# UMich-CURLY/SE3ET

Measured on AMD Instinct MI355X. Metric: point-cloud pairs/sec (fwd), SE3ET-E 5k-pt pairs, higher is better.
Workload: dtype f32

## Files before the change

include/se3et_hip.h:

```cpp
#ifndef SE3ET_HIP_H_
#define SE3ET_HIP_H_

#include <stddef.h>
#include <stdint.h>

#ifdef __cplusplus
extern "C" {
#endif

#define SE3_OK 0
#define SE3_ERR_INVALID_ARG 1
#define SE3_ERR_UNSUPPORTED 2
#define SE3_ERR_LAUNCH 3
#define SE3_ERR_WORKSPACE 4

#define SE3_MAX_BATCH 32
#define SE3_MAX_NEIGHBOR_LIMIT 64

const char* se3_version(void);
const char* se3_last_error(void);
void se3_debug_set_sinkhorn_variant(int variant);
unsigned long long se3_debug_dense_saturated_rows(int reset);
unsigned long long se3_debug_attention_saturated(int reset);
void se3_debug_kernel_timing(int enable);
int se3_debug_kernel_timing_collect_ex(float* microseconds, int* tags, double* aux, int capacity);

int se3_radius_neighbors(const float* q_points, int64_t nq, const float* s_points, int64_t ns,
                         const int64_t* q_lengths_host, const int64_t* s_lengths_host, int batch, float radius,
                         int limit, int64_t* neighbors, int32_t* max_count, void* stream);

int se3_neighbor_table_trim(const int64_t* full, int64_t rows, int full_width, int width, const int64_t* pair_row_ends_host,
                            const int* pair_widths_host, int num_pairs, int64_t* out, void* stream);
size_t se3_radius_grid_workspace_bytes(int64_t ns, int batch);
int se3_radius_grid_build(const float* s_points, int64_t ns, const int64_t* s_lengths_host, int batch, float radius,
                          void* workspace, size_t workspace_bytes, void* stream);
int se3_radius_neighbors_grid(const float* q_points, int64_t nq, const int64_t* q_lengths_host, const int64_t* s_lengths_host,
                              int64_t ns, int batch, const void* grid_workspace, float radius, int limit, int64_t* neighbors,
                              int32_t* max_count, int max_count_is_zero, void* stream);

int se3_radius_count_hist(const float* q_points, int64_t nq, const float* s_points, int64_t ns, const int64_t* q_lengths_host,
                          const int64_t* s_lengths_host, int batch, float radius, const void* grid_workspace, int hist_n,
                          const int* slot_of_cloud_host, int num_slots, int32_t* hist, int32_t* dropped, int32_t* max_count, void* stream);

int se3_radius_neighbors_ties(const float* q_points, int64_t nq, const float* s_points, int64_t ns, const int64_t* q_lengths_host,
                              const int64_t* s_lengths_host, int batch, float radius, int limit, int64_t* neighbors, int32_t* max_count,
                              int32_t* tie_rows, int32_t* tie_count, void* stream);
int se3_radius_neighbors_grid_ties(const float* q_points, int64_t nq, const int64_t* q_lengths_host, const int64_t* s_lengths_host,
                                   int64_t ns, int batch, const void* grid_workspace, float radius, int limit, int64_t* neighbors,
                                   int32_t* max_count, int max_count_is_zero, int32_t* tie_rows, int32_t* tie_count, void* stream);
size_t se3_kdtree_max_bytes(int64_t ns, int batch);
int se3_kdtree_build_host(const float* s_points_host, int64_t ns, const int64_t* s_lengths_host, int batch, void* tree_host, size_t capacity,
                          size_t* used_bytes);
size_t se3_radius_tie_scratch_bytes(int64_t num_tie_rows, int max_hits);
int se3_radius_neighbors_tie_order(const float* q_points, int64_t nq, const float* s_points, int64_t ns, const int64_t* q_lengths_host,
                                   const int64_t* s_lengths_host, int batch, const void* tree_dev, float radius, int limit,
                                   const int32_t* tie_rows, int64_t num_tie_rows, int max_hits, void* scratch, size_t scratch_bytes,
                                   int64_t* neighbors, void* stream);
int se3_debug_radius_tie_order_host(const float* q_points, int64_t nq, const float* s_points, int64_t ns, const int64_t* q_lengths,
                                    const int64_t* s_lengths, int batch, const void* tree_host, float radius, int limit,
                                    const int32_t* tie_rows, int64_t num_tie_rows, int max_hits, int64_t* neighbors, int* overflowed);
int64_t se3_debug_std_sort_host(const unsigned long long* keys, int64_t n, int mode);

size_t se3_grid_subsample_workspace_bytes(int64_t n, int batch);
int se3_grid_subsample(const float* points, const float* normals, int64_t n, const int64_t* lengths_host, int batch,
                       float voxel_size, float* s_points, float* s_normals, int64_t* s_lengths, void* workspace,
                       size_t workspace_bytes, void* stream);
int se3_grid_subsample_dev(const float* points, const float* normals, int64_t n_rows, const int64_t* lengths_dev, int batch,
                           float voxel_size, float* s_points, float* s_normals, int64_t* s_lengths, void* workspace,
                           size_t workspace_bytes, void* stream);

int se3_log_sinkhorn_fwd(const float* scores, const uint8_t* row_masks, const uint8_t* col_masks, const float* alpha,
                         int batch, int rows, int cols, int iterations, float inf, float* out, void* stream);
int se3_log_sinkhorn_bwd(const float* scores, const uint8_t* row_masks, const uint8_t* col_masks, const float* alpha,
                         const float* grad_out, int batch, int rows, int cols, int iterations, float inf, float* grad_scores,
                         float* grad_alpha_partial, void* stream);

size_t se3_group_norm_workspace_bytes(int64_t rows, int channels, int groups);
int se3_group_norm_fwd(const float* x, const float* x_bias, const float* residual, const float* weight, const float* bias,
                       int64_t rows, int channels, int groups, float eps, int apply_leaky_relu, float slope, float* out,
                       void* workspace, size_t workspace_bytes, void* stream);

int se3_group_norm_segments_fwd(const float* x, const float* x_bias, const float* residual, const float* weight,
                                const float* bias, int64_t rows, int channels, int groups,
                                const int64_t* segment_row_offsets_host, int num_segments, float eps, int apply_leaky_relu,
                                float slope, float* out, void* workspace, size_t workspace_bytes, void* stream);
size_t se3_group_norm_bwd_workspace_bytes(int channels);
int se3_group_norm_segments_bwd(const float* x, const float* x_bias, const float* residual, const float* weight, const float* bias,
                                const float* grad_out, int64_t rows, int channels, int groups, const int64_t* segment_row_offsets_host,
                                int num_segments, float eps, int apply_leaky_relu, float slope, float* grad_x, float* grad_residual,
                                float* grad_params, void* workspace, size_t workspace_bytes, void* stream);

size_t se3_group_norm_stats_workspace_bytes(int channels);
int se3_group_norm_stats(const float* x, const float* in_affine, float in_slope, const float* x_bias, const float* weight, const float* bias,
                         int64_t rows, int channels, int groups, const int64_t* segment_row_offsets_host, int num_segments, float eps,
                         float* affine_out, void* workspace, size_t workspace_bytes, void* stream);
int se3_group_norm_apply(const float* x, const float* affine_a, float slope_a, const float* affine_b, float slope_b, const float* residual,
                         const float* residual_affine, float final_slope, int64_t rows, int channels,
                         const int64_t* segment_row_offsets_host, int num_segments, int blocked_layout, float* out, void* stream);
int se3_group_norm_apply_amax(const float* x, const float* affine_a, float slope_a, const float* affine_b, float slope_b, const float* residual,
                              const float* residual_affine, float final_slope, int64_t rows, int channels,
                              const int64_t* segment_row_offsets_host, int num_segments, int blocked_layout, float* out, float* amax_out,
                              void* stream);
size_t se3_dense_norm_workspace_bytes(int groups);
int se3_dense_norm_fwd(const float* x, int64_t rows, int in_features, const float* in_affine_a, float in_slope_a, const float* in_affine_b,
                       float in_slope_b, const void* weight_pieces, int out_features, const float* linear_bias, const float* norm_weight,
// ... 556 lines not shown
```

se3et_amd/csrc/dense_norm.hip:

```cpp
#include "common.h"
#include "group_norm.h"

namespace {

using f16x8 = __attribute__((ext_vector_type(8))) _Float16;
using f16x4 = __attribute__((ext_vector_type(4))) _Float16;
using f32x16 = __attribute__((ext_vector_type(16))) float;
using f32x4 = __attribute__((ext_vector_type(4))) float;
using u32x4 = __attribute__((ext_vector_type(4))) unsigned;
using i32x4 = __attribute__((ext_vector_type(4))) int;

__device__ unsigned long long g_dense_saturated_rows = 0;

template <int CTRL>
__device__ __forceinline__ float dpp_f32(float v) {
  return __builtin_bit_cast(float, __builtin_amdgcn_update_dpp(0, __builtin_bit_cast(int, v), CTRL, 0xf, 0xf, true));
}

constexpr int kHeaderB = 256;
constexpr int kRowB = 80;

struct DenseArgs {
  const float* x;
  const float* in_affine[2];
  float in_slope[2];
  int K, N, NCT;
  const u32x4* Wf;
  const float* hdr;
  float* out;
  float* part;
  int* counters;
  const float* xb;
  const float* gw;
  const float* gb;
  float* affine;
  int groups;
  float eps;
  SegTable T;
  const float* affine1;
  const float* residual;
  const float* x2;
  int K2;
  const u32x4* Wf2;
  const float* hdr2;
  const float* affine2;
  float final_slope;
  int x_rs, out_rs;
  int t_rows;
  int t_ld;
  int seg_steps;
  long long seg_stride;
};


struct StepPos {
  int tile, kk;
};
template <int WM, int WN, int RT, int CT, int MODE>
__global__ __launch_bounds__(256, MODE == 3 ? 2 : 3) void dense_norm_kernel(const DenseArgs a) {
  static_assert(WM * WN == 4, "4 waves");
  constexpr int TR = 32 * RT * WM, BN = 32 * CT * WN, U = TR / 32;
  constexpr int kPieceB = TR * kRowB, kBufB = 2 * kPieceB;
  constexpr bool kStats = MODE <= 1, kDual = MODE == 3, kPlain = MODE >= 4;
  __shared__ __align__(16) unsigned char lds[2 * kBufB];
  __shared__ __align__(16) int row_exp[2][TR];
  __shared__ __align__(16) int row_exp_step[2][TR];
  __shared__ int row_run[TR];
  __shared__ int row_scl[2];
  extern __shared__ __align__(16) float aff[];
  const int tid = threadIdx.x, lane = tid & 63, wave = __builtin_amdgcn_readfirstlane(tid >> 6);
  const int wm = wave / WN, wn = wave % WN;
  const int i32 = lane & 31, h = lane >> 5;
  const int K = a.K, N = a.N;
  const int K2 = kDual ? a.K2 : 32;
  const int XS = kPlain ? a.x_rs : K, OS = kPlain ? a.out_rs : N;
  long long r0, r1;
  chunk_rows(a.T, blockIdx.x, r0, r1);
  if (r1 < r0) r1 = r0;
  const int seg = seg_of_chunk(a.T, blockIdx.x);
  int cb0 = a.T.chunk_begin[0], cb1 = a.T.chunk_begin[1];
#pragma unroll
  for (int i = 1; i < kGNMaxSegments; i++)
    if (seg == i) {
// ... 396 lines not shown
  StepPos pr{0, 0}, ps{0, 0}, pm{0, 0};
  request(pr, ra);
  advance(pr);
  request(pr, rb);
  advance(pr);
  __syncthreads();
  stage(0, ps, ra);
  advance(ps);
#pragma unroll
  for (int j = 0; j < U; j++) ra[j] = rb[j];
  request(pr, rb);
  advance(pr);
  __syncthreads();
  if constexpr (WD == 1) {
#pragma unroll 1
    for (int s = 0; s < total; s++) {
      multiply(s & 1, pm, bq[0]);
      advance(pm);
      stage((s + 1) & 1, ps, ra);
      advance(ps);
#pragma unroll
      for (int j = 0; j < U; j++) ra[j] = rb[j];
      request(pr, rb);
      advance(pr);
      __syncthreads();
    }
  } else {
#pragma unroll 1
    for (int s = 0; s < total; s += WD) {
#pragma unroll
      for (int j = 0; j < WD; j++) {
        if (s + j >= total) break;
        multiply(j & 1, pm, bq[j]);
        advance(pm);
        stage((j + 1) & 1, ps, ra);
        advance(ps);
#pragma unroll
        for (int u = 0; u < U; u++) ra[u] = rb[u];
        request(pr, rb);
        advance(pr);
        __syncthreads();
      }
    }
  }
  if constexpr (!kStats) return;
  __syncthreads();
  const int cpg = N / a.groups;
  WF* sh = reinterpret_cast<WF*>(lds);
  if (a.xb)
#pragma unroll
    for (int c = 0; c < CT; c++) run[c].mean += a.xb[(ct0 + c) * 32 + i32];
  if (h == 0)
#pragma unroll
    for (int c = 0; c < CT; c++) sh[(wave * CT + c) * 32 + i32] = run[c];
  __syncthreads();
  if (wm == 0)
#pragma unroll
    for (int c = 0; c < CT; c++) {
      WF w = run[c];
      for (int m = 1; m < WM; m++) w = wf_merge(w, sh[((m * WN + wn) * CT + c) * 32 + i32]);
      for (int d = 1; d < cpg; d <<= 1) {
        const WF o = {__shfl_xor(w.n, d), __shfl_xor(w.mean, d), __shfl_xor(w.m2, d)};
        w = wf_merge(w, o);
      }
      const int col = (ct0 + c) * 32 + i32;
      if (h == 0 && (col & (cpg - 1)) == 0) gn_store_partial(a.part + ((int64_t)blockIdx.x * a.groups + col / cpg) * 3, w);
    }
  if (!gn_last_arrival(a.counters + seg * kGNMaxColumnBlocks + blockIdx.y, cb1 - cb0)) return;
  const int gpb = BN / cpg;
  gn_finalize_groups(a.part, a.groups, cb0, cb1, blockIdx.y * gpb, gpb, cpg, a.xb, a.gw, a.gb, a.eps, a.affine + (size_t)seg * 2 * N, N);
}

constexpr int kTargetChunks = 768;

}

extern "C" unsigned long long se3_debug_dense_saturated_rows(int reset) {
  unsigned long long n = 0;
  if (hipMemcpyFromSymbol(&n, HIP_SYMBOL(g_dense_saturated_rows), sizeof(n)) != hipSuccess) return ~0ull;
  if (reset) {
    const unsigned long long zero = 0;
    (void)hipMemcpyToSymbol(HIP_SYMBOL(g_dense_saturated_rows), &zero, sizeof(zero));
  }
  return n;
}

constexpr size_t kCounterB = kGNCounterB;

extern "C" size_t se3_dense_norm_workspace_bytes(int groups) {
  return kCounterB + (size_t)(kGNMaxChunks + kGNMaxSegments) * (groups > 0 ? groups : 1) * 3 * sizeof(float);
}

namespace {
int dense_chunks(int64_t rows, int N, const int64_t* segment_row_offsets_host, int num_segments, SegTable& T, int& TR, int& BN, int& ncb,
                 bool given = false) {
  if (!given) {
    TR = N >= 256 ? 64 : 128;
    BN = N >= 256 ? 256 : N;
  }
  ncb = (N + BN - 1) / BN;
  T = SegTable{};
  T.n = num_segments;
  T.quantum = TR;
  int64_t tiles = 0;
  for (int s = 0; s < num_segments; s++) {
    const int64_t b0 = num_segments == 1 ? 0 : segment_row_offsets_host[s], b1 = num_segments == 1 ? rows : segment_row_offsets_host[s + 1];
    if (!(b1 > b0 && b0 >= 0 && b1 <= rows)) return -1;
    tiles += se3_cdiv(b1 - b0, TR);
  }
  int64_t want = kTargetChunks / ncb;
  if (want > kGNMaxChunks - num_segments) want = kGNMaxChunks - num_segments;
  if (want < 1) want = 1;
  int64_t tiles_per_chunk = se3_cdiv(tiles, want);
  for (int s = 0; s < num_segments; s++) {
    const int64_t b0 = num_segments == 1 ? 0 : segment_row_offsets_host[s], b1 = num_segments == 1 ? rows : segment_row_offsets_host[s + 1];
    const int64_t need = se3_cdiv(se3_cdiv(b1 - b0, TR), 256);
    if (need > tiles_per_chunk) tiles_per_chunk = need;
  }
  int chunks = 0;
  for (int s = 0; s < num_segments; s++) {
    const int64_t b0 = num_segments == 1 ? 0 : segment_row_offsets_host[s], b1 = num_segments == 1 ? rows : segment_row_offsets_host[s + 1];
    T.row_begin[s] = b0;
    T.row_begin[s + 1] = b1;
    T.chunk_begin[s] = chunks;
    chunks += (int)se3_cdiv(se3_cdiv(b1 - b0, TR), tiles_per_chunk);
    T.chunk_begin[s + 1] = chunks;
  }
  if (!(T.row_begin[0] == 0 && T.row_begin[num_segments] == rows && chunks <= kGNMaxChunks + kGNMaxSegments)) return -1;
  return chunks;
}

template <int MODE>
void dense_launch(const DenseArgs& a, int N, dim3 grid, size_t dyn, hipStream_t st) {
  if (N >= 256) dense_norm_kernel<1, 4, 2, 2, MODE><<<grid, 256, dyn, st>>>(a);
  else if (N == 128) dense_norm_kernel<2, 2, 2, 2, MODE><<<grid, 256, dyn, st>>>(a);
  else if (N == 64) dense_norm_kernel<4, 1, 1, 2, MODE><<<grid, 256, dyn, st>>>(a);
  else dense_norm_kernel<4, 1, 1, 1, MODE><<<grid, 256, dyn, st>>>(a);
}
}

extern "C" int se3_dense_norm_fwd(const float* x, int64_t rows, int in_features, const float* in_affine_a, float in_slope_a,
                                  const float* in_affine_b, float in_slope_b, const void* weight_pieces, int out_features,
                                  const float* linear_bias, const float* norm_weight, const float* norm_bias, int groups, float eps,
                                  const int64_t* segment_row_offsets_host, int num_segments, float* out, float* affine_out, void* workspace,
                                  size_t workspace_bytes, void* stream) {
  SE3_REQUIRE(x && weight_pieces && norm_weight && norm_bias && affine_out && workspace, SE3_ERR_INVALID_ARG, "dense_norm: null pointer");
  const int K = in_features, N = out_features;
  SE3_REQUIRE(K >= 32 && K <= 1024 && (K & (K - 1)) == 0 && N >= 32 && N % 32 == 0 && (N < 256 ? (N & (N - 1)) == 0 : N % 256 == 0),
              SE3_ERR_UNSUPPORTED, "dense_norm: %d -> %d features (in: a power of two 32..1024; out: 32, 64, 128 or a multiple of 256)", K, N);
  SE3_REQUIRE(rows >= 1 && groups >= 1 && N % groups == 0, SE3_ERR_INVALID_ARG, "dense_norm: rows %lld groups %d", (long long)rows, groups);
  {
    const int cpg = N / groups;
    SE3_REQUIRE(cpg <= 32 && (cpg & (cpg - 1)) == 0 && N / (N >= 256 ? 256 : N) <= kGNMaxColumnBlocks, SE3_ERR_UNSUPPORTED,
                "dense_norm: %d channels per group (a power of two <= 32), %d output features (<= %d)", cpg, N, 256 * kGNMaxColumnBlocks);
  }
  SE3_REQUIRE(num_segments >= 1 && num_segments <= kGNMaxSegments && (num_segments == 1 || segment_row_offsets_host), SE3_ERR_UNSUPPORTED,
              "dense_norm: %d segments (1..%d)", num_segments, kGNMaxSegments);
  SE3_REQUIRE(((uintptr_t)x & 15) == 0 && (in_affine_a || !in_affine_b), SE3_ERR_INVALID_ARG, "dense_norm: x must be 16-byte aligned; stage b needs stage a");
  SE3_REQUIRE(in_slope_a >= 0.f && in_slope_a <= 1.f && in_slope_b >= 0.f && in_slope_b <= 1.f, SE3_ERR_INVALID_ARG, "dense_norm: LeakyReLU slopes must lie in [0, 1]");
  SE3_REQUIRE(workspace_bytes >= se3_dense_norm_workspace_bytes(groups), SE3_ERR_WORKSPACE, "dense_norm: workspace too small");
  SegTable T;
  int TR, BN, ncb;
  const int chunks = dense_chunks(rows, N, segment_row_offsets_host, num_segments, T, TR, BN, ncb);
  SE3_REQUIRE(chunks > 0, SE3_ERR_INVALID_ARG, "dense_norm: the segments must be non-empty, ascending and cover all %lld rows", (long long)rows);
  DenseArgs a{};
  a.x = x;
  a.in_affine[0] = in_affine_a;
  a.in_affine[1] = in_affine_b;
  a.in_slope[0] = in_slope_a;
  a.in_slope[1] = in_slope_b;
  a.K = K;
  a.N = N;
  a.NCT = (N + 63) / 64 * 2;
  a.hdr = static_cast<const float*>(weight_pieces);
  a.Wf = reinterpret_cast<const u32x4*>(static_cast<const unsigned char*>(weight_pieces) + kHeaderB);
  a.out = out;
  a.counters = static_cast<int*>(workspace);
  a.part = reinterpret_cast<float*>(static_cast<unsigned char*>(workspace) + kCounterB);
  a.xb = linear_bias;
  a.gw = norm_weight;
  a.gb = norm_bias;
  a.affine = affine_out;
  a.groups = groups;
  a.eps = eps;
  a.T = T;
  const size_t dyn = (size_t)((in_affine_a != nullptr) + (in_affine_b != nullptr)) * 2 * K * sizeof(float);
  hipStream_t st = (hipStream_t)stream;
  const dim3 grid((unsigned)chunks, (unsigned)ncb);
  if (out != nullptr) dense_launch<0>(a, N, grid, dyn, st);
  else dense_launch<1>(a, N, grid, dyn, st);
  SE3_CHECK_LAUNCH("dense_norm");
  return SE3_OK;
}

extern "C" int se3_dense_residual_fwd(const float* x, int64_t rows, int in_features, const float* in_affine_a, float in_slope_a,
                                      const float* in_affine_b, float in_slope_b, const void* weight_pieces, const float* affine,
                                      const float* x2, int in_features2, const void* weight_pieces2, const float* affine2,
                                      const float* residual, int out_features, float final_slope, const int64_t* segment_row_offsets_host,
                                      int num_segments, float* out, void* stream) {
  SE3_REQUIRE(x && weight_pieces && affine && out, SE3_ERR_INVALID_ARG, "dense_residual: null pointer");
  const int K = in_features, N = out_features, K2 = in_features2;
  SE3_REQUIRE(K >= 32 && K <= 1024 && (K & (K - 1)) == 0 && N >= 32 && N % 32 == 0 && (N < 256 ? (N & (N - 1)) == 0 : N % 256 == 0),
              SE3_ERR_UNSUPPORTED, "dense_residual: %d -> %d features (in: a power of two 32..1024; out: 32, 64, 128 or a multiple of 256)", K, N);
  SE3_REQUIRE(!(x2 && residual), SE3_ERR_INVALID_ARG, "dense_residual: a residual tensor OR a shortcut layer");
  SE3_REQUIRE(!x2 || (weight_pieces2 && affine2 && K2 >= 32 && K2 <= 1024 && (K2 & (K2 - 1)) == 0 && ((uintptr_t)x2 & 15) == 0), SE3_ERR_UNSUPPORTED,
              "dense_residual: shortcut layer with %d input features (a power of two 32..1024, 16-byte aligned rows)", K2);
  SE3_REQUIRE(rows >= 1 && num_segments >= 1 && num_segments <= kGNMaxSegments && (num_segments == 1 || segment_row_offsets_host), SE3_ERR_UNSUPPORTED,
              "dense_residual: rows %lld, %d segments (1..%d)", (long long)rows, num_segments, kGNMaxSegments);
  SE3_REQUIRE(((uintptr_t)x & 15) == 0 && (in_affine_a || !in_affine_b), SE3_ERR_INVALID_ARG, "dense_residual: x must be 16-byte aligned; stage b needs stage a");
  SE3_REQUIRE(in_slope_a >= 0.f && in_slope_a <= 1.f && in_slope_b >= 0.f && in_slope_b <= 1.f && final_slope >= 0.f && final_slope <= 1.f, SE3_ERR_INVALID_ARG,
              "dense_residual: LeakyReLU slopes must lie in [0, 1]");
  SegTable T;
  int TR, BN, ncb;
  const int chunks = dense_chunks(rows, N, segment_row_offsets_host, num_segments, T, TR, BN, ncb);
  SE3_REQUIRE(chunks > 0, SE3_ERR_INVALID_ARG, "dense_residual: the segments must be non-empty, ascending and cover all %lld rows", (long long)rows);
  DenseArgs a{};
  a.x = x;
  a.in_affine[0] = in_affine_a;
  a.in_affine[1] = in_affine_b;
  a.in_slope[0] = in_slope_a;
  a.in_slope[1] = in_slope_b;
  a.K = K;
  a.N = N;
  a.NCT = (N + 63) / 64 * 2;
  a.hdr = static_cast<const float*>(weight_pieces);
  a.Wf = reinterpret_cast<const u32x4*>(static_cast<const unsigned char*>(weight_pieces) + kHeaderB);
  a.out = out;
  a.T = T;
  a.affine1 = affine;
  a.residual = residual;
  a.final_slope = final_slope;
  const size_t dyn = (size_t)((in_affine_a != nullptr) + (in_affine_b != nullptr)) * 2 * K * sizeof(float);
  hipStream_t st = (hipStream_t)stream;
  const dim3 grid((unsigned)chunks, (unsigned)ncb);
  if (x2 != nullptr) {
    a.x2 = x2;
    a.K2 = K2;
    a.hdr2 = static_cast<const float*>(weight_pieces2);
    a.Wf2 = reinterpret_cast<const u32x4*>(static_cast<const unsigned char*>(weight_pieces2) + kHeaderB);
    a.affine2 = affine2;
    dense_launch<3>(a, N, grid, dyn, st);
  } else {
    dense_launch<2>(a, N, grid, dyn, st);
  }
  SE3_CHECK_LAUNCH("dense_residual");
  return SE3_OK;
}


namespace {
template <int WM, int WN, int RT, int CT>
void plain_launch(const DenseArgs& a, bool transposed, dim3 grid, hipStream_t st) {
  if (transposed) dense_norm_kernel<WM, WN, RT, CT, 5><<<grid, 256, 0, st>>>(a);
  else dense_norm_kernel<WM, WN, RT, CT, 4><<<grid, 256, 0, st>>>(a);
}
int linear_stream_one(const float* x, int64_t rows, int K, int64_t x_rs, const void* weight_pieces, const float* bias, int N, int relu, float* out,
                      int64_t out_rs, int t_rows, int64_t t_ld, void* stream, int seg_channels = 0, int64_t seg_stride = 0) {
  SE3_REQUIRE(x && weight_pieces && out, SE3_ERR_INVALID_ARG, "linear_stream: null pointer");
  SE3_REQUIRE(K > 0 && K % 32 == 0 && N > 0, SE3_ERR_UNSUPPORTED, "linear_stream: in_features %d must be a multiple of 32", K);
  SE3_REQUIRE(x_rs >= 4 && x_rs % 4 == 0 && ((uintptr_t)x & 15) == 0 && rows * x_rs < (1ll << 29), SE3_ERR_INVALID_ARG,
              "linear_stream: x rows must be 16-byte aligned, row stride %lld, below 2 GB", (long long)x_rs);
  const bool transposed = t_rows > 0;
  if (transposed)
    SE3_REQUIRE(t_rows % 4 == 0 && rows % t_rows == 0 && t_ld >= t_rows && t_ld % 4 == 0 && ((uintptr_t)out & 15) == 0 &&
                    (rows / t_rows) * N * t_ld < (1ll << 29),
                SE3_ERR_INVALID_ARG, "linear_stream: transposed output blocks of %d rows (a multiple of 4 dividing %lld), leading dimension %lld",
                t_rows, (long long)rows, (long long)t_ld);
  else
    SE3_REQUIRE(out_rs >= N && rows * out_rs < (1ll << 29), SE3_ERR_INVALID_ARG, "linear_stream: out row stride %lld", (long long)out_rs);
  if (rows == 0) return SE3_OK;
  int TR, BN, cfg;
  const int64_t rt64 = se3_cdiv(rows, 64);
  if (N > 128) {
    if (rt64 * se3_cdiv(N, 256) >= 512) { TR = 64; BN = 256; cfg = 0; }
    else if (rt64 * se3_cdiv(N, 128) >= 320 || N % 128 > 64) { TR = 64; BN = 128; cfg = 1; }
    else { TR = 64; BN = 64; cfg = 2; }
  } else if (N > 64) { TR = rt64 >= 512 ? 128 : 64; BN = 128; cfg = rt64 >= 512 ? 3 : 1; }
  else if (N > 32) { TR = rt64 >= 512 ? 128 : 64; BN = 64; cfg = rt64 >= 512 ? 4 : 2; }
  else { TR = 128; BN = 32; cfg = 5; }
  if (transposed && cfg == 3) { TR = 64; cfg = 1; }
  SegTable T;
  int ncb;
  const int chunks = dense_chunks(rows, N, nullptr, 1, T, TR, BN, ncb, true);
  SE3_REQUIRE(chunks > 0, SE3_ERR_INVALID_ARG, "linear_stream: %lld rows", (long long)rows);
  DenseArgs a{};
  a.x = x;
  a.K = K;
  a.N = N;
  a.NCT = (N + 63) / 64 * 2;
  a.hdr = static_cast<const float*>(weight_pieces);
  a.Wf = reinterpret_cast<const u32x4*>(static_cast<const unsigned char*>(weight_pieces) + kHeaderB);
  a.out = out;
  a.xb = bias;
  a.T = T;
  a.final_slope = relu ? 0.f : 1.f;
  a.x_rs = (int)x_rs;
  a.out_rs = (int)out_rs;
  a.t_rows = t_rows;
  a.t_ld = (int)t_ld;
  if (seg_channels > 0) {
    SE3_REQUIRE(seg_channels % 32 == 0 && K % seg_channels == 0 && seg_stride >= rows * x_rs && (K / seg_channels) * seg_stride < (1ll << 29),
                SE3_ERR_INVALID_ARG, "linear_stream: %d input channels in segments of %d", K, seg_channels);
    a.seg_steps = seg_channels / 32;
    a.seg_stride = seg_stride;
  }
  hipStream_t st = (hipStream_t)stream;
  const dim3 grid((unsigned)chunks, (unsigned)ncb);
  switch (cfg) {
    case 0: plain_launch<1, 4, 2, 2>(a, transposed, grid, st); break;
    case 1: plain_launch<2, 2, 1, 2>(a, transposed, grid, st); break;
    case 2: plain_launch<2, 2, 1, 1>(a, transposed, grid, st); break;
    case 3: plain_launch<2, 2, 2, 2>(a, transposed, grid, st); break;
    case 4: plain_launch<4, 1, 1, 2>(a, transposed, grid, st); break;
    default: plain_launch<4, 1, 1, 1>(a, transposed, grid, st); break;
  }
  SE3_CHECK_LAUNCH("linear_stream");
  return SE3_OK;
}

int linear_stream(const float* x, int64_t rows, int K, int64_t x_rs, const void* weight_pieces, const float* bias, int N, int relu, float* out,
                  int64_t out_rs, int t_rows, int64_t t_ld, void* stream, int seg_channels = 0, int64_t seg_stride = 0) {
  const int64_t lim = (1ll << 29) - 1;
  const bool transposed = t_rows > 0;
  const bool fits = rows >= 0 && x_rs > 0 && rows * x_rs <= lim &&
                    (transposed ? (rows / t_rows) * (int64_t)N * t_ld <= lim : rows * (out_rs > N ? out_rs : (int64_t)N) <= lim);
  if (fits || seg_channels > 0 || !x || !out || N <= 0) return linear_stream_one(x, rows, K, x_rs, weight_pieces, bias, N, relu, out, out_rs, t_rows, t_ld, stream, seg_channels, seg_stride);
  int64_t step;
  if (transposed) {
    SE3_REQUIRE(rows % t_rows == 0 && t_ld >= t_rows, SE3_ERR_INVALID_ARG, "linear_stream: transposed output blocks of %d rows", t_rows);
    const int64_t per_block = std::max((int64_t)t_rows * x_rs, (int64_t)N * t_ld);
    SE3_REQUIRE(per_block <= lim, SE3_ERR_UNSUPPORTED, "linear_stream: one transposed block of %d rows exceeds 2 GB", t_rows);
    step = lim / per_block * t_rows;
  } else {
    SE3_REQUIRE(out_rs >= N, SE3_ERR_INVALID_ARG, "linear_stream: out row stride %lld", (long long)out_rs);
    step = lim / std::max(x_rs, out_rs) / 256 * 256;
    SE3_REQUIRE(step > 0, SE3_ERR_UNSUPPORTED, "linear_stream: row strides %lld / %lld too large", (long long)x_rs, (long long)out_rs);
  }
  for (int64_t r0 = 0; r0 < rows; r0 += step) {
    const int64_t n = std::min(step, rows - r0);
    float* o = transposed ? out + (r0 / t_rows) * (int64_t)N * t_ld : out + r0 * out_rs;
    const int rc = linear_stream_one(x + r0 * x_rs, n, K, x_rs, weight_pieces, bias, N, relu, o, out_rs, t_rows, t_ld, stream);
    if (rc != SE3_OK) return rc;
  }
  return SE3_OK;
}
}

extern "C" int se3_linear_stream(const float* x, int64_t rows, int in_features, int64_t x_row_stride, const void* weight_pieces, const float* bias,
                                 int out_features, int apply_relu, float* out, int64_t out_row_stride, void* stream) {
  return linear_stream(x, rows, in_features, x_row_stride, weight_pieces, bias, out_features, apply_relu, out, out_row_stride, 0, 0, stream);
}

extern "C" int se3_linear_stream_transposed(const float* x, int64_t rows, int in_features, int64_t x_row_stride, const void* weight_pieces,
                                            const float* bias, int out_features, int block_rows, float* out_t, int64_t ld, void* stream) {
  SE3_REQUIRE(block_rows > 0, SE3_ERR_INVALID_ARG, "linear_stream_transposed: block_rows %d", block_rows);
  return linear_stream(x, rows, in_features, x_row_stride, weight_pieces, bias, out_features, 0, out_t, 0, block_rows, ld, stream);
}


extern "C" int se3_linear_stream_segments(const float* x, int64_t rows, int in_features, int seg_channels, int64_t seg_stride,
                                          const void* weight_pieces, const float* bias, int out_features, int apply_relu, float* out,
                                          int64_t out_row_stride, void* stream) {
  SE3_REQUIRE(seg_channels > 0, SE3_ERR_INVALID_ARG, "linear_stream_segments: seg_channels %d", seg_channels);
  return linear_stream(x, rows, in_features, seg_channels, weight_pieces, bias, out_features, apply_relu, out, out_row_stride, 0, 0, stream,
                       seg_channels, seg_stride);
}
```

se3et_amd/ops.py:

```python
import ctypes
import os
import threading

import torch

from .caches import CACHE_EPOCH, Derived, Workspace, _Shared, also_clear, clear_caches, clear_weight_caches, validate_weight_caches
from ._lib import CONSTANTS, ENUMS, check, lib
from .stacking import PAIR_MAX_PAIRS, device_offsets, exclusive_offsets, to_device


_HAS_BLAS_SWITCH = hasattr(torch.backends.cuda, 'preferred_blas_library')
if _HAS_BLAS_SWITCH:
    torch.backends.cuda.preferred_blas_library('cublas')
_BLAS_SWITCH_LOCK = threading.Lock()
_BIG_GEMM_FLOP = 2.0e9


def mm(a, b):
    big = 2.0 * a.shape[0] * a.shape[1] * b.shape[1] > _BIG_GEMM_FLOP
    if _HAS_BLAS_SWITCH and big and (b.stride(-1) == 1 or a.shape[1] <= 32):
        with _BLAS_SWITCH_LOCK:
            torch.backends.cuda.preferred_blas_library('cublaslt')
            try:
                return torch.mm(a, b)
            finally:
                torch.backends.cuda.preferred_blas_library('cublas')
    if _HAS_BLAS_SWITCH and threading.active_count() > 1:
        with _BLAS_SWITCH_LOCK:
            return torch.mm(a, b)
    return torch.mm(a, b)


LINEAR_F16_MIN_ROWS, LINEAR_F16_MIN_K = 20000, 256
_linear_pieces = Derived(512, weights=True)


def _linear_weight_pieces(weight, stream):
    N, K = weight.shape
    owner = weight._base if weight._base is not None else weight
    key = (weight.data_ptr(), N, K, weight.stride(0), weight.device.index)
    Wp = _linear_pieces.lookup(owner, key)
    if Wp is not None:
        return Wp
    Wp = torch.empty((lib().se3_linear_weight_pieces_bytes(N, K),), dtype=torch.uint8, device=weight.device)
    w = weight.detach()
    w = w if w.is_contiguous() else w.contiguous()
    check(lib().se3_linear_split_weights_f16(w.data_ptr(), N, K, Wp.data_ptr(), stream), 'se3_linear_split_weights_f16')
    return _linear_pieces.store(owner, key, Wp, fingerprint_of=(weight,))


_stacked_weights = Derived(128, weights=True)


def stacked_weight(weight, groups):
    key = (weight.data_ptr(), tuple(weight.shape), int(groups), weight.device.index)
    W = _stacked_weights.lookup(weight, key)
    if W is not None:
        return W
    with torch.no_grad():
        W = torch.cat([weight.detach()] * int(groups), 1).contiguous()
    return _stacked_weights.store(weight, key, W, fingerprint_of=(weight,))


def linear_f16_ok(x, weight):
    if torch.is_grad_enabled() and (x.requires_grad or weight.requires_grad):
        return False
    if not (x.is_cuda and x.dtype == torch.float32 and weight.dtype == torch.float32 and weight.dim() == 2 and weight.is_contiguous()):
        return False
    K = weight.shape[1]
    rows = x.numel() // max(x.shape[-1], 1)
    return (x.shape[-1] == K and K % 32 == 0 and K >= LINEAR_F16_MIN_K and rows >= LINEAR_F16_MIN_ROWS and x.is_contiguous()
            and x.data_ptr() % 16 == 0)


def linear_f16(x, weight, bias=None, relu=False):
    stream = _stream()
    N, K = weight.shape
    rows = x.numel() // K
    Wp = _linear_weight_pieces(weight, stream)
    out = torch.empty(x.shape[:-1] + (N,), dtype=torch.float32, device=x.device)
    b = None if bias is None else _req(bias.detach().contiguous(), torch.float32, 'bias', 1)
    check(lib().se3_linear_f16(x.data_ptr(), rows, K, K, Wp.data_ptr(), None if b is None else b.data_ptr(), N, 1 if relu else 0,
                               out.data_ptr(), N, stream), 'se3_linear_f16')
    return out


def dense_saturated_rows(reset=True):
    return int(lib().se3_debug_dense_saturated_rows(1 if reset else 0))


def attention_saturated(reset=True):
    return int(lib().se3_debug_attention_saturated(1 if reset else 0))


def linear_stream_ok(x, weight):
    if torch.is_grad_enabled() and (x.requires_grad or weight.requires_grad):
        return False
    if not (x.is_cuda and x.dtype == torch.float32 and weight.dtype == torch.float32 and weight.dim() == 2 and weight.stride(1) == 1):
        return False
    K = weight.shape[1]
    return x.shape[-1] == K and K % 32 == 0 and x.stride(-1) == 1 and x.data_ptr() % 16 == 0 and (x.is_contiguous() or (x.dim() == 2 and x.stride(0) % 4 == 0))


def linear_stream(x, weight, bias=None, relu=False, out=None):
    stream = _stream()
    N, K = weight.shape
    rows = x.numel() // K
    x_rs = x.stride(0) if (x.dim() == 2 and not x.is_contiguous()) else K
    Wp = _linear_weight_pieces(weight, stream)
    if out is None:
        out = torch.empty(x.shape[:-1] + (N,), dtype=torch.float32, device=x.device)
        out_rs = N
    else:
        if out.dim() != 2 or out.shape[0] != rows or out.shape[1] != N or out.stride(1) != 1 or out.dtype != torch.float32:
            raise RuntimeError('linear_stream: out must be a (rows, N) float32 view with unit column stride')
        out_rs = out.stride(0)
    b = None if bias is None else _req(bias.detach().contiguous(), torch.float32, 'bias', 1)
    check(lib().se3_linear_stream(x.data_ptr(), rows, K, x_rs, Wp.data_ptr(), None if b is None else b.data_ptr(), N, 1 if relu else 0,
                                  out.data_ptr(), out_rs, stream), 'se3_linear_stream')
    return out


def linear_stream_transposed(x, weight, bias, ld=None):
    A, R, K = x.shape
    N = weight.shape[0]
    ld = R if ld is None else int(ld)
    stream = _stream()
    Wp = _linear_weight_pieces(weight, stream)
    out = torch.empty((A, N, ld), dtype=torch.float32, device=x.device)
    b = None if bias is None else _req(bias.detach().contiguous(), torch.float32, 'bias', 1)
    check(lib().se3_linear_stream_transposed(x.data_ptr(), A * R, K, K, Wp.data_ptr(), None if b is None else b.data_ptr(), N, R, out.data_ptr(), ld,
                                             stream), 'se3_linear_stream_transposed')
    return out


TIMING_TAG = None
KERNEL_TIMINGS = None
_TIMING_LOCK = threading.Lock()


class _timed:
    def __init__(self, name, nbytes, kind=None):
        self.name, self.nbytes, self.kind = name, nbytes, kind

    def __enter__(self):
        if KERNEL_TIMINGS is not None:
            self.e0, self.e1 = torch.cuda.Event(enable_timing=True), torch.cuda.Event(enable_timing=True)
            self.e0.record()

    def __exit__(self, *exc):
        if KERNEL_TIMINGS is not None:
            self.e1.record()
            KERNEL_TIMINGS.setdefault(self.name, []).append((self.e0, self.e1, self.nbytes))
            if self.kind is not None:
                KERNEL_TIMINGS.setdefault(self.name + '/' + self.kind, []).append((self.e0, self.e1, self.nbytes))
            if TIMING_TAG is not None:
                KERNEL_TIMINGS.setdefault(self.name + '@' + TIMING_TAG, []).append((self.e0, self.e1, self.nbytes))
        return False


_raw_stream = getattr(torch._C, '_cuda_getCurrentRawStream', None)


def _stream():
    if _raw_stream is not None:
        return ctypes.c_void_p(_raw_stream(torch.cuda.current_device()))
    return ctypes.c_void_p(torch.cuda.current_stream().cuda_stream)


def _req(t, dtype, name, ndim=None):
    if not torch.is_tensor(t):
# ... 2419 lines not shown
```

Before: 468.8.

## Add persistent tall-tile split-f16 MFMA kernel for large linear_stream GEMMs

Adds a dense_tall kernel used when a linear_stream call has at least 16384 rows and K and N are both at least 256. Each block works through a contiguous run of rows with a 256x256 tile, double-buffering x and weight fragments in LDS and software-pipelining global loads, staging and MFMA across steps. It keeps the hi/lo f16 split with per-row exponent rescaling for out-of-range values. The goal is more weight reuse and fewer launched blocks on tall GEMMs, at the cost of a large LDS and register footprint that may limit occupancy. A debug variant switch allows forcing either path.

```diff
diff --git a/include/se3et_hip.h b/include/se3et_hip.h
--- a/include/se3et_hip.h
+++ b/include/se3et_hip.h
@@ -21,6 +21,7 @@
 const char* se3_last_error(void);
 void se3_debug_set_sinkhorn_variant(int variant);
 unsigned long long se3_debug_dense_saturated_rows(int reset);
+void se3_debug_set_dense_plain_variant(int variant);
 unsigned long long se3_debug_attention_saturated(int reset);
 void se3_debug_kernel_timing(int enable);
 int se3_debug_kernel_timing_collect_ex(float* microseconds, int* tags, double* aux, int capacity);
diff --git a/se3et_amd/csrc/dense_norm.hip b/se3et_amd/csrc/dense_norm.hip
--- a/se3et_amd/csrc/dense_norm.hip
+++ b/se3et_amd/csrc/dense_norm.hip
@@ -1,4 +1,5 @@
 #include "common.h"
+#include "dense_tall.h"
 #include "group_norm.h"
 
 namespace {
@@ -561,7 +562,9 @@
     const unsigned long long zero = 0;
     (void)hipMemcpyToSymbol(HIP_SYMBOL(g_dense_saturated_rows), &zero, sizeof(zero));
   }
-  return n;
+  unsigned long long tall = 0;
+  if (!dense_tall_saturated_rows(reset, &tall)) return ~0ull;
+  return n + tall;
 }
 
 constexpr size_t kCounterB = kGNCounterB;
@@ -728,6 +731,12 @@
 
 
 namespace {
+int g_dense_plain_variant = 0;
+
+bool tall_policy(int64_t rows, int K, int N) {
+  return rows >= 16384 && K >= 256 && N >= 256;
+}
+
 template <int WM, int WN, int RT, int CT>
 void plain_launch(const DenseArgs& a, bool transposed, dim3 grid, hipStream_t st) {
   if (transposed) dense_norm_kernel<WM, WN, RT, CT, 5><<<grid, 256, 0, st>>>(a);
@@ -758,6 +767,24 @@
   else if (N > 32) { TR = rt64 >= 512 ? 128 : 64; BN = 64; cfg = rt64 >= 512 ? 4 : 2; }
   else { TR = 128; BN = 32; cfg = 5; }
   if (transposed && cfg == 3) { TR = 64; cfg = 1; }
+  const bool tall_ok = !transposed && seg_channels == 0 && x_rs >= K && N > 128 && x_rs <= (1 << 20) && out_rs <= (1 << 20);
+  if (tall_ok && g_dense_plain_variant != 1 && (g_dense_plain_variant == 2 || tall_policy(rows, K, N))) {
+    DenseTallArgs t{};
+    t.x = x;
+    t.hdr = static_cast<const float*>(weight_pieces);
+    t.Wf = static_cast<const unsigned char*>(weight_pieces) + kHeaderB;
+    t.bias = bias;
+    t.out = out;
+    t.rows = rows;
+    t.K = K;
+    t.N = N;
+    t.NCT = (N + 63) / 64 * 2;
+    t.x_rs = (int)x_rs;
+    t.out_rs = (int)out_rs;
+    t.final_slope = relu ? 0.f : 1.f;
+    t.count_bn = BN;
+    return dense_tall_launch(t, (hipStream_t)stream);
+  }
   SegTable T;
   int ncb;
   const int chunks = dense_chunks(rows, N, nullptr, 1, T, TR, BN, ncb, true);
@@ -825,6 +852,8 @@
 }
 }
 
+extern "C" void se3_debug_set_dense_plain_variant(int variant) { g_dense_plain_variant = variant; }
+
 extern "C" int se3_linear_stream(const float* x, int64_t rows, int in_features, int64_t x_row_stride, const void* weight_pieces, const float* bias,
                                  int out_features, int apply_relu, float* out, int64_t out_row_stride, void* stream) {
   return linear_stream(x, rows, in_features, x_row_stride, weight_pieces, bias, out_features, apply_relu, out, out_row_stride, 0, 0, stream);
diff --git a/se3et_amd/csrc/dense_tall.h b/se3et_amd/csrc/dense_tall.h
--- /dev/null
+++ b/se3et_amd/csrc/dense_tall.h
@@ -0,0 +1,18 @@
+#pragma once
+#include "common.h"
+
+struct DenseTallArgs {
+  const float* x;
+  const void* Wf;
+  const float* hdr;
+  const float* bias;
+  float* out;
+  long long rows;
+  int K, N, NCT;
+  int x_rs, out_rs;
+  float final_slope;
+  int count_bn;
+};
+
+int dense_tall_launch(const DenseTallArgs& a, hipStream_t stream);
+bool dense_tall_saturated_rows(int reset, unsigned long long* n);
diff --git a/se3et_amd/csrc/dense_tall.hip b/se3et_amd/csrc/dense_tall.hip
--- /dev/null
+++ b/se3et_amd/csrc/dense_tall.hip
@@ -0,0 +1,318 @@
+#include "dense_tall.h"
+
+namespace {
+
+using f16x8 = __attribute__((ext_vector_type(8))) _Float16;
+using f16x4 = __attribute__((ext_vector_type(4))) _Float16;
+using f32x16 = __attribute__((ext_vector_type(16))) float;
+using f32x4 = __attribute__((ext_vector_type(4))) float;
+using u32x4 = __attribute__((ext_vector_type(4))) unsigned;
+using i32x4 = __attribute__((ext_vector_type(4))) int;
+
+__device__ unsigned long long g_dense_tall_saturated_rows = 0;
+
+constexpr int kRowB = 80;
+constexpr int kWM = 4, kWN = 2, kRT = 2, kCT = 4;
+constexpr int kTR = 32 * kRT * kWM, kBN = 32 * kCT * kWN;
+constexpr int kThreads = 64 * kWM * kWN;
+constexpr int kU = kTR / 64;
+constexpr int kPieceB = kTR * kRowB, kABufB = 2 * kPieceB;
+constexpr int kWFragB = 64 * 16;
+constexpr int kWBufB = 2 * (kBN / 32) * 2 * kWFragB;
+constexpr int kWU = kWBufB / (kThreads * 16);
+static_assert(kWU == 4 && kU == 4, "staging maps below");
+
+struct StepPos {
+  int tile, kk;
+};
+
+__global__ __launch_bounds__(kThreads) void dense_tall_kernel(const DenseTallArgs a, const long long rows_per) {
+  __shared__ __align__(16) unsigned char lds[2 * kABufB + 2 * kWBufB];
+  __shared__ __align__(16) int row_exp[2][kTR];
+  __shared__ __align__(16) int row_exp_step[2][kTR];
+  __shared__ int row_run[kTR];
+  __shared__ int row_scl[2];
+  unsigned char* const wlds = lds + 2 * kABufB;
+  const int tid = threadIdx.x, lane = tid & 63, wave = __builtin_amdgcn_readfirstlane(tid >> 6);
+  const int wm = wave / kWN, wn = wave % kWN;
+  const int i32 = lane & 31, h = lane >> 5;
+  const int K = a.K, N = a.N, XS = a.x_rs, OS = a.out_rs;
+  const long long r0 = (long long)blockIdx.x * rows_per;
+  const long long r1 = r0 + rows_per < a.rows ? r0 + rows_per : a.rows;
+  if (r1 <= r0) return;
+  if (tid < 2) row_scl[tid] = -1;
+  for (int i = tid; i < 2 * kTR; i += kThreads) row_exp_step[0][i] = -1;
+  const int nkt = K >> 5;
+  const int nrows = (int)(r1 - r0);
+  const int ntiles = (nrows + kTR - 1) / kTR;
+  const int total = ntiles * nkt;
+  auto advance = [&](StepPos& p) {
+    p.kk++;
+    if (p.kk == nkt) {
+      p.kk = 0;
+      p.tile++;
+    }
+  };
+  const int q = tid & 7, urow = 32 * wave + (lane >> 3);
+  const int xoff = (urow * XS + 4 * q) * 4, jstep = 8 * XS * 4;
+  const float* xbase = a.x + r0 * XS;
+  bool plain_rows = true;
+  auto request = [&](const StepPos& p, f32x4 (&v)[kU]) {
+    const int left = p.tile < ntiles ? nrows - p.tile * kTR : 0;
+    const __amdgpu_buffer_rsrc_t xrs = __builtin_amdgcn_make_buffer_rsrc(const_cast<float*>(xbase + (long long)(left > 0 ? p.tile : 0) * kTR * XS), 0,
+                                                                         left * XS * 4, 0x00020000);
+    const int soff = p.kk * 32 * 4;
+#pragma unroll
+    for (int j = 0; j < kU; j++) v[j] = __builtin_bit_cast(f32x4, __builtin_amdgcn_raw_buffer_load_b128(xrs, xoff + j * jstep, soff, 0));
+  };
+  auto stage = [&](int buf, const StepPos& p, const f32x4 (&v)[kU]) {
+    const bool first_step = p.kk == 0, last_step = p.kk == nkt - 1;
+    unsigned long long odd = 0;
+#pragma unroll
+    for (int j = 0; j < kU; j++) {
+      const f32x4 t = v[j];
+      const float m = fmaxf(fmaxf(__builtin_fabsf(t[0]), __builtin_fabsf(t[1])), fmaxf(__builtin_fabsf(t[2]), __builtin_fabsf(t[3])));
+      odd |= __builtin_amdgcn_ballot_w64(!(m < (first_step ? 128.f : 32768.f)));
+      unsigned long long ge = __builtin_amdgcn_ballot_w64(m >= 0.0625f);
+      ge |= ge >> 4;
+      ge |= ge >> 2;
+      ge |= ge >> 1;
+      odd |= first_step ? (~ge & 0x0101010101010101ull) : 0ull;
+    }
+    if (__builtin_expect(odd == 0 && (plain_rows || first_step), 1)) {
+#pragma unroll
+      for (int j = 0; j < kU; j++) {
+          f16x4 hi, lo;
+#pragma unroll
+        for (int e = 0; e < 4; e++) {
+          hi[e] = (_Float16)v[j][e];
+          lo[e] = (_Float16)(v[j][e] - (float)hi[e]);
+        }
+        unsigned char* dst = lds + buf * kABufB + (urow + 8 * j) * kRowB + q * 8;
+        *reinterpret_cast<f16x4*>(dst) = hi;
+        *reinterpret_cast<f16x4*>(dst + kPieceB) = lo;
+      }
+      plain_rows = true;
+      return;
+    }
+    bool any_scaled = false;
+    int saturated = 0;
+#pragma unroll 1
+    for (int j = 0; j < kU; j++) {
+      f32x4 t = v[0];
+#pragma unroll
+      for (int jj = 1; jj < kU; jj++) t = j == jj ? v[jj] : t;
+      float m = fmaxf(fmaxf(__builtin_fabsf(t[0]), __builtin_fabsf(t[1])), fmaxf(__builtin_fabsf(t[2]), __builtin_fabsf(t[3])));
+      const bool nan = (t[0] != t[0]) | (t[1] != t[1]) | (t[2] != t[2]) | (t[3] != t[3]);
+      m = nan ? __builtin_bit_cast(float, 0x7fc00000) : m;
+      int mb = __builtin_bit_cast(int, m);
+      mb = max(mb, __builtin_amdgcn_update_dpp(0, mb, 0xB1, 0xf, 0xf, true));
+      mb = max(mb, __builtin_amdgcn_update_dpp(0, mb, 0x4E, 0xf, 0xf, true));
+      mb = max(mb, __builtin_amdgcn_update_dpp(0, mb, 0x141, 0xf, 0xf, true));
+      const int e_here = (mb >> 23) & 0xff;
+      const int row = urow + 8 * j;
+      int e_row;
+      if (first_step)
+        e_row = ((e_here >= 123 && e_here <= 133) || e_here == 0) ? 141 : (e_here >= 255 ? 141 : min(e_here + 8, 254));
+      else
+        e_row = plain_rows ? 141 : row_run[row];
+      if (first_step && q == 0) row_run[row] = e_row;
+      const bool sat = e_here > e_row;
+      f16x4 hi, lo;
+#pragma unroll
+      for (int e = 0; e < 4; e++) {
+        float te = __builtin_ldexpf(t[e], 141 - e_row);
+        te = fminf(fmaxf(te, -65000.f), 65000.f);
+        te = (__float_as_uint(t[e]) & 0x7f800000u) == 0x7f800000u ? __builtin_bit_cast(float, 0x7fc00000) : te;
+        hi[e] = (_Float16)te;
+        lo[e] = (_Float16)(te - (float)hi[e]);
+      }
+      unsigned char* dst = lds + buf * kABufB + row * kRowB + q * 8;
+      *reinterpret_cast<f16x4*>(dst) = hi;
+      *reinterpret_cast<f16x4*>(dst + kPieceB) = lo;
+      if (last_step && e_row != 141 && q == 0) {
+        row_exp[buf][row] = e_row - 141;
+        row_exp_step[buf][row] = p.tile * nkt + p.kk;
+      }
+      saturated += (sat && q == 0) ? 1 : 0;
+      any_scaled |= e_row != 141;
+    }
+    const bool w_scaled = __builtin_amdgcn_ballot_w64(any_scaled) != 0;
+    plain_rows = !w_scaled;
+    if (last_step && w_scaled && lane == 0) row_scl[buf] = p.tile * nkt + p.kk;
+    if (saturated) {
+      const int per = kBN / a.count_bn, blocks = (N + a.count_bn - 1) / a.count_bn - (int)blockIdx.y * per;
+      atomicAdd(&g_dense_tall_saturated_rows, (unsigned long long)(saturated * (blocks < per ? blocks : per)));
+    }
+  };
+  const u32x4* Wf = reinterpret_cast<const u32x4*>(a.Wf);
+  const int ctb = blockIdx.y * (kBN / 32);
+  int wsrc[2];
+#pragma unroll
+  for (int i = 0; i < 2; i++) {
+    const int ct = ctb + 4 * i + (tid >> 7);
+    wsrc[i] = (ct < a.NCT ? ct : a.NCT - 1) * 128 + (tid & 127);
+  }
+  const int wstep = a.NCT * 128;
+  auto request_w = [&](int kk, u32x4 (&w)[kWU]) {
+    const u32x4* base = Wf + (int64_t)(2 * kk) * wstep;
+#pragma unroll
+    for (int i = 0; i < kWU; i++) w[i] = base[(i >> 1) * wstep + wsrc[i & 1]];
+  };
+  auto stage_w = [&](int buf, const u32x4 (&w)[kWU]) {
+#pragma unroll
+    for (int i = 0; i < kWU; i++) *reinterpret_cast<u32x4*>(wlds + buf * kWBufB + (i * kThreads + tid) * 16) = w[i];
+  };
+  const int a_read = (wm * (kRT * 32) + i32) * kRowB + h * 16;
+  const int w_read = wn * kCT * 2 * kWFragB + lane * 16;
+  const int ct0 = ctb + wn * kCT;
+  const bool cols_live = ct0 * 32 < N;
+  const float inv_scale = a.hdr[0];
+  float bs[kCT];
+#pragma unroll
+  for (int c = 0; c < kCT; c++) {
+    const int col = (ct0 + c) * 32 + i32;
+    bs[c] = (a.bias != nullptr && col < N) ? a.bias[col] : 0.f;
+  }
+  f32x16 acc[kRT][kCT];
+#pragma unroll
+  for (int r = 0; r < kRT; r++)
+#pragma unroll
+    for (int c = 0; c < kCT; c++)
+#pragma unroll
+      for (int v = 0; v < 16; v++) acc[r][c][v] = 0.f;
+
+  auto multiply = [&](int buf, const StepPos& p) {
+    const long long trow0 = r0 + (long long)p.tile * kTR + wm * (kRT * 32);
+    const int rows_here = (int)(r1 - trow0 < kRT * 32 ? (r1 - trow0 > 0 ? r1 - trow0 : 0) : kRT * 32);
+    if (rows_here == 0 || !cols_live) return;
+    const unsigned char* img = lds + buf * kABufB + a_read;
+    const unsigned char* wimg = wlds + buf * kWBufB + w_read;
+#pragma unroll
+    for (int ks = 0; ks < 2; ks++) {
+      f16x8 av[kRT][2], b0[kCT], b1[kCT];
+#pragma unroll
+      for (int r = 0; r < kRT; r++) {
+        av[r][0] = *reinterpret_cast<const f16x8*>(img + r * 32 * kRowB + ks * 32);
+        av[r][1] = *reinterpret_cast<const f16x8*>(img + r * 32 * kRowB + ks * 32 + kPieceB);
+      }
+#pragma unroll
+      for (int c = 0; c < kCT; c++) {
+        b0[c] = *reinterpret_cast<const f16x8*>(wimg + ((ks * 8 + c) * 2 + 0) * kWFragB);
+        b1[c] = *reinterpret_cast<const f16x8*>(wimg + ((ks * 8 + c) * 2 + 1) * kWFragB);
+      }
+#pragma unroll
+      for (int c = 0; c < kCT; c++)
+#pragma unroll
+        for (int r = 0; r < kRT; r++) acc[r][c] = __builtin_amdgcn_mfma_f32_32x32x16_f16(av[r][1], b0[c], acc[r][c], 0, 0, 0);
+#pragma unroll
+      for (int c = 0; c < kCT; c++)
+#pragma unroll
+        for (int r = 0; r < kRT; r++) acc[r][c] = __builtin_amdgcn_mfma_f32_32x32x16_f16(av[r][0], b1[c], acc[r][c], 0, 0, 0);
+#pragma unroll
+      for (int c = 0; c < kCT; c++)
+#pragma unroll
+        for (int r = 0; r < kRT; r++) acc[r][c] = __builtin_amdgcn_mfma_f32_32x32x16_f16(av[r][0], b0[c], acc[r][c], 0, 0, 0);
+    }
+  };
+  auto finish = [&](int buf, const StepPos& p) {
+    if (p.kk != nkt - 1) return;
+    const long long trow0 = r0 + (long long)p.tile * kTR + wm * (kRT * 32);
+    const int rows_here = (int)(r1 - trow0 < kRT * 32 ? (r1 - trow0 > 0 ? r1 - trow0 : 0) : kRT * 32);
+    if (rows_here == 0 || !cols_live) return;
+    if (__builtin_expect(row_scl[buf] == p.tile * nkt + p.kk, 0)) {
+      const int step_id = p.tile * nkt + p.kk;
+#pragma unroll
+      for (int r = 0; r < kRT; r++)
+#pragma unroll
+        for (int g = 0; g < 4; g++) {
+          const int base = (wm * kRT + r) * 32 + 8 * g + 4 * h;
+          const i32x4 tag = *reinterpret_cast<const i32x4*>(&row_exp_step[buf][base]);
+          const i32x4 ex = *reinterpret_cast<const i32x4*>(&row_exp[buf][base]);
+#pragma unroll
+          for (int j = 0; j < 4; j++) {
+            const int ev = tag[j] == step_id ? ex[j] : 0;
+#pragma unroll
+            for (int c = 0; c < kCT; c++) acc[r][c][4 * g + j] = __builtin_ldexpf(acc[r][c][4 * g + j], ev);
+          }
+        }
+    }
+    const __amdgpu_buffer_rsrc_t ors = __builtin_amdgcn_make_buffer_rsrc(a.out + trow0 * OS, 0, ((rows_here - 1) * OS + N) * 4, 0x00020000);
+    const int left = rows_here - 4 * h;
+#pragma unroll
+    for (int c = 0; c < kCT; c++) {
+      const int col = (ct0 + c) * 32 + i32;
+      const int col_off = col < N ? (4 * h * OS + col) * 4 : 0x7ffffff0;
+#pragma unroll
+      for (int r = 0; r < kRT; r++)
+#pragma unroll
+        for (int v = 0; v < 16; v++) {
+          const int rr = r * 32 + (v & 3) + 8 * (v >> 2);
+          float val = acc[r][c][v] * inv_scale + bs[c];
+          val = fmaxf(val, val * a.final_slope);
+          __builtin_amdgcn_raw_buffer_store_b32(__builtin_bit_cast(unsigned, val), ors, rr < left ? col_off : 0x7ffffff0, rr * OS * 4, 0);
+          acc[r][c][v] = 0.f;
+        }
+    }
+  };
+
+  f32x4 ra[kU], rb[kU];
+  u32x4 wq[kWU];
+  StepPos pr{0, 0}, ps{0, 0}, pm{0, 0};
+  request_w(0, wq);
+  request(pr, ra);
+  advance(pr);
+  request(pr, rb);
+  advance(pr);
+  __syncthreads();
+  stage_w(0, wq);
+  stage(0, ps, ra);
+  advance(ps);
+  request_w(ps.kk, wq);
+  request(pr, ra);
+  advance(pr);
+  __syncthreads();
+  const bool late = wave >= 4;
+  auto step = [&](int buf, f32x4 (&r)[kU]) {
+    if (!late) multiply(buf, pm);
+    if (ps.tile * kTR + 32 * wave < nrows) stage(buf ^ 1, ps, r);
+    stage_w(buf ^ 1, wq);
+    advance(ps);
+    request_w(ps.kk, wq);
+    request(pr, r);
+    advance(pr);
+    if (late) multiply(buf, pm);
+    finish(buf, pm);
+    advance(pm);
+    __syncthreads();
+  };
+#pragma unroll 1
+  for (int s = 0; s < total; s += 2) {
+    step(0, rb);
+    if (s + 1 >= total) break;
+    step(1, ra);
+  }
+}
+
+}
+
+bool dense_tall_saturated_rows(int reset, unsigned long long* n) {
+  if (hipMemcpyFromSymbol(n, HIP_SYMBOL(g_dense_tall_saturated_rows), sizeof(*n)) != hipSuccess) return false;
+  if (reset) {
+    const unsigned long long zero = 0;
+    (void)hipMemcpyToSymbol(HIP_SYMBOL(g_dense_tall_saturated_rows), &zero, sizeof(zero));
+  }
+  return true;
+}
+
+int dense_tall_launch(const DenseTallArgs& a, hipStream_t stream) {
+  const int ncb = (a.N + kBN - 1) / kBN;
+  int64_t want = 256 / ncb;
+  if (want < 1) want = 1;
+  const int64_t units = se3_cdiv(a.rows, 64);
+  const int64_t chunks = units < want ? units : want;
+  const long long rows_per = se3_cdiv(a.rows, chunks);
+  dense_tall_kernel<<<dim3((unsigned)chunks, (unsigned)ncb), kThreads, 0, stream>>>(a, rows_per);
+  SE3_CHECK_LAUNCH("linear_stream (tall tile)");
+  return SE3_OK;
+}
diff --git a/se3et_amd/ops.py b/se3et_amd/ops.py
--- a/se3et_amd/ops.py
+++ b/se3et_amd/ops.py
@@ -87,6 +87,10 @@
 
 def dense_saturated_rows(reset=True):
     return int(lib().se3_debug_dense_saturated_rows(1 if reset else 0))
+
+
+def set_dense_plain_variant(variant):
+    lib().se3_debug_set_dense_plain_variant(int(variant))
 
 
 def attention_saturated(reset=True):
```

Result: faster. 474.4, median of 6 (+1.2%).
